# firstbatchxyz/dnet

Measured on AMD Instinct MI355X. Metric: output tokens/sec (whole node), qwen-2.5-32b int8 pipelined ring, higher is better.
Workload: dtype int8-g128 weights (bf16 compute); 1 GPU; model=qwen-2.5-32b, global_batch=64, seq_len=128, gen_len=178, parallelism=ring-pp1, microbatches=1, mb_size=64, layers=64

## Files before the change

dnet_amd/ops/csrc/gemm_m16.hip.cpp:

```cpp
#include "common.h"

namespace dnet {

using bf16x8 = __attribute__((ext_vector_type(8))) __bf16;
using f32x4 = __attribute__((ext_vector_type(4))) float;

__device__ __forceinline__ bf16x8 deq8(const int8_t* q, const float s) {
  bf16x8 b;
#pragma unroll
  for (int j = 0; j < 8; ++j) b[j] = (__bf16)((float)q[j] * s);
  return b;
}

__device__ __forceinline__ bf16x8 deq4(const uint8_t* qb, const float s) {
  bf16x8 b;
#pragma unroll
  for (int j = 0; j < 4; ++j) {
    const int byte = qb[j];
    b[2 * j] = (__bf16)((float)((byte & 0xF) - 8) * s);
    b[2 * j + 1] = (__bf16)((float)((byte >> 4) - 8) * s);
  }
  return b;
}

__device__ __forceinline__ float splitk_grid(const float v) {
  return rintf(v * 65536.0f) * (1.0f / 65536.0f);
}

template <int QBITS, int MT>
__global__ void gemm_m16_kernel(const short* __restrict__ x,
                                const void* __restrict__ w,
                                const short* __restrict__ scales,
                                const short* __restrict__ bias,
                                short* __restrict__ out,
                                float* __restrict__ out_f32,
                                const int M, const int K, const int N,
                                const int G, const int splitk,
                                const int exact) {
  constexpr int XT = 1024 / MT;
  constexpr int SE = XT + 8;
  __shared__ short x_lds[16 * MT * SE];
  const int wave = threadIdx.x / kWave;
  const int lane = threadIdx.x & (kWave - 1);
  const int n0 = (blockIdx.x * 4 + wave) * 16;
  const int row = lane & 15;
  const int ks = (lane >> 4) * 8;
  const int n_w = min(n0 + row, N - 1);

  const int pairs = K / 64;
  int p_begin, p_end;
  if (QBITS == 4) {
    const int quads = K / 128;
    const int qq = quads / splitk;
    p_begin = blockIdx.y * qq * 2;
    p_end = (blockIdx.y == splitk - 1) ? quads * 2 : p_begin + qq * 2;
  } else {
    const int pp = pairs / splitk;
    p_begin = blockIdx.y * pp;
    p_end = (blockIdx.y == splitk - 1) ? pairs : p_begin + pp;
  }
  const int woff = (lane >> 4) * 16;

  f32x4 acc[MT][2];
#pragma unroll
  for (int t = 0; t < MT; ++t)
#pragma unroll
    for (int u = 0; u < 2; ++u) acc[t][u] = {0.f, 0.f, 0.f, 0.f};

  const int8_t* wrow_q = (const int8_t*)w + (int64_t)n_w * K;
  const uint8_t* wrow_q4 = (const uint8_t*)w + (int64_t)n_w * (K / 2);
  const short* wrow_b = (const short*)w + (int64_t)n_w * K;
  const short* srow = QBITS < 16 ? scales + (int64_t)n_w * (K / G) : nullptr;

  for (int k0 = p_begin * 64; k0 < p_end * 64; k0 += XT) {
    const int tk = min(XT, p_end * 64 - k0);
    asm volatile("s_waitcnt lgkmcnt(0)" ::: "memory");
    asm volatile("s_barrier" ::: "memory");
    for (int idx = threadIdx.x; idx < 16 * MT * (tk / 8); idx += 256) {
      const int r = idx / (tk / 8);
      const int vec = idx % (tk / 8);
      *reinterpret_cast<short8*>(&x_lds[r * SE + vec * 8]) =
          *reinterpret_cast<const short8*>(
              &x[(int64_t)min(r, M - 1) * K + k0 + vec * 8]);
    }
    asm volatile("s_waitcnt lgkmcnt(0)" ::: "memory");
    asm volatile("s_barrier" ::: "memory");
    const short* arow = &x_lds[row * SE];
    int pl = 0;
    const int pl_end = tk / 64;
    for (; pl + 4 <= pl_end; pl += 4) {
      int4 wq8[4];
      int4 wq4[2];
      bf16x8 wb[4][2];
      float sv[4];
      if (QBITS == 8) {
#pragma unroll
        for (int u = 0; u < 4; ++u) {
          const int p = (k0 / 64) + pl + u;
          wq8[u] = *reinterpret_cast<const int4*>(&wrow_q[p * 64 + woff]);
          sv[u] = bits2f(srow[(p * 64) / G]);
        }
      } else if (QBITS == 4) {
#pragma unroll
        for (int v = 0; v < 2; ++v) {
          const int quad = ((k0 / 64) + pl) / 2 + v;
          wq4[v] = *reinterpret_cast<const int4*>(&wrow_q4[quad * 64 + woff]);
          sv[v] = bits2f(srow[(quad * 128) / G]);
        }
      } else {
#pragma unroll
        for (int u = 0; u < 4; ++u) {
          const int p = (k0 / 64) + pl + u;
          wb[u][0] = *reinterpret_cast<const bf16x8*>(&wrow_b[p * 64 + ks]);
          wb[u][1] = *reinterpret_cast<const bf16x8*>(
              &wrow_b[p * 64 + 32 + ks]);
        }
      }
#pragma unroll
      for (int u = 0; u < 4; ++u) {
        bf16x8 b0, b1;
        if (QBITS == 8) {
          const int8_t* q8 = reinterpret_cast<const int8_t*>(&wq8[u]);
          b0 = deq8(q8, sv[u]);
          b1 = deq8(q8 + 8, sv[u]);
        } else if (QBITS == 4) {
          const uint8_t* q4 =
              reinterpret_cast<const uint8_t*>(&wq4[u / 2]) + (u & 1) * 8;
          b0 = deq4(q4, sv[u / 2]);
          b1 = deq4(q4 + 4, sv[u / 2]);
        } else {
          b0 = wb[u][0];
          b1 = wb[u][1];
        }
#pragma unroll
        for (int t = 0; t < MT; ++t) {
          const short* at = arow + t * 16 * SE;
          const bf16x8 a0 =
              *reinterpret_cast<const bf16x8*>(&at[(pl + u) * 64 + ks]);
          const bf16x8 a1 =
              *reinterpret_cast<const bf16x8*>(&at[(pl + u) * 64 + 32 + ks]);
          acc[t][0] = __builtin_amdgcn_mfma_f32_16x16x32_bf16(
              a0, b0, acc[t][0], 0, 0, 0);
          acc[t][1] = __builtin_amdgcn_mfma_f32_16x16x32_bf16(
              a1, b1, acc[t][1], 0, 0, 0);
        }
      }
    }
    for (; pl < pl_end; ++pl) {
      const int p = (k0 / 64) + pl;
      bf16x8 b0, b1;
      if (QBITS == 8) {
        const int4 wq = *reinterpret_cast<const int4*>(&wrow_q[p * 64 + woff]);
        const int8_t* q8 = reinterpret_cast<const int8_t*>(&wq);
        const float sv = bits2f(srow[(p * 64) / G]);
        b0 = deq8(q8, sv);
        b1 = deq8(q8 + 8, sv);
      } else if (QBITS == 4) {
        const int quad = p / 2;
        const int half = p & 1;
        const int2 wq = *reinterpret_cast<const int2*>(
            &wrow_q4[quad * 64 + woff + half * 8]);
        const uint8_t* q4 = reinterpret_cast<const uint8_t*>(&wq);
        const float sv = bits2f(srow[(quad * 128) / G]);
        b0 = deq4(q4, sv);
        b1 = deq4(q4 + 4, sv);
      } else {
        b0 = *reinterpret_cast<const bf16x8*>(&wrow_b[p * 64 + ks]);
        b1 = *reinterpret_cast<const bf16x8*>(&wrow_b[p * 64 + 32 + ks]);
      }
#pragma unroll
      for (int t = 0; t < MT; ++t) {
        const short* at = arow + t * 16 * SE;
        const bf16x8 a0 = *reinterpret_cast<const bf16x8*>(&at[pl * 64 + ks]);
        const bf16x8 a1 = *reinterpret_cast<const bf16x8*>(&at[pl * 64 + 32 + ks]);
        acc[t][0] = __builtin_amdgcn_mfma_f32_16x16x32_bf16(a0, b0, acc[t][0],
                                                            0, 0, 0);
        acc[t][1] = __builtin_amdgcn_mfma_f32_16x16x32_bf16(a1, b1, acc[t][1],
                                                            0, 0, 0);
      }
    }
  }

  const int n = n0 + (lane & 15);
  if (n >= N) return;
#pragma unroll
  for (int t = 0; t < MT; ++t) {
    const f32x4 a2 = acc[t][0] + acc[t][1];
#pragma unroll
    for (int r = 0; r < 4; ++r) {
      const int m = t * 16 + (lane >> 4) * 4 + r;
      if (m >= M) continue;
      if (splitk > 1) {
        atomicAdd(out_f32 + (int64_t)m * N + n,
                  exact ? splitk_grid(a2[r]) : a2[r]);
      } else {
        float v = a2[r];
        if (bias != nullptr) v += bits2f(bias[n]);
        out[(int64_t)m * N + n] = f2bits(v);
      }
    }
  }
}


using i32x4 = __attribute__((ext_vector_type(4))) int;

template <int QBITS, int NSC>
struct WSet {
  i32x4 w[QBITS == 8 ? 4 : 2];
  unsigned s[NSC];
};

template <int QBITS, int NSC>
__device__ __forceinline__ void wset_load(WSet<QBITS, NSC>& o,
                                          const void* wb, const short* sb) {
  if constexpr (QBITS == 8 && NSC == 2) {
    asm volatile(
        "global_load_dwordx4 %0, %6, off\n\t"
        "global_load_dwordx4 %1, %6, off offset:64\n\t"
        "global_load_dwordx4 %2, %6, off offset:128\n\t"
        "global_load_dwordx4 %3, %6, off offset:192\n\t"
        "global_load_ushort %4, %7, off\n\t"
        "global_load_ushort %5, %7, off offset:2\n\t"
        "s_waitcnt vmcnt(0)"
        : "=&v"(o.w[0]), "=&v"(o.w[1]), "=&v"(o.w[2]), "=&v"(o.w[3]),
          "=&v"(o.s[0]), "=&v"(o.s[1])
        : "v"(wb), "v"(sb)
        : "memory");
  } else if constexpr (QBITS == 8 && NSC == 4) {
    asm volatile(
        "global_load_dwordx4 %0, %8, off\n\t"
        "global_load_dwordx4 %1, %8, off offset:64\n\t"
        "global_load_dwordx4 %2, %8, off offset:128\n\t"
        "global_load_dwordx4 %3, %8, off offset:192\n\t"
        "global_load_ushort %4, %9, off\n\t"
        "global_load_ushort %5, %9, off offset:2\n\t"
        "global_load_ushort %6, %9, off offset:4\n\t"
        "global_load_ushort %7, %9, off offset:6\n\t"
        "s_waitcnt vmcnt(0)"
        : "=&v"(o.w[0]), "=&v"(o.w[1]), "=&v"(o.w[2]), "=&v"(o.w[3]),
          "=&v"(o.s[0]), "=&v"(o.s[1]), "=&v"(o.s[2]), "=&v"(o.s[3])
        : "v"(wb), "v"(sb)
        : "memory");
  } else {
    static_assert(QBITS == 4 && NSC == 2, "unsupported stream variant");
    asm volatile(
        "global_load_dwordx4 %0, %4, off\n\t"
        "global_load_dwordx4 %1, %4, off offset:64\n\t"
        "global_load_ushort %2, %5, off\n\t"
        "global_load_ushort %3, %5, off offset:2\n\t"
        "s_waitcnt vmcnt(0)"
        : "=&v"(o.w[0]), "=&v"(o.w[1]), "=&v"(o.s[0]), "=&v"(o.s[1])
        : "v"(wb), "v"(sb)
        : "memory");
  }
}

template <int QBITS, int NSC>
struct WSet2 {
  i32x4 w[QBITS == 8 ? 8 : 4];
  unsigned s[2 * NSC];
};

template <int QBITS, int NSC>
__device__ __forceinline__ void wset_load2(WSet2<QBITS, NSC>& o,
                                           const void* wb, const short* sb) {
  if constexpr (QBITS == 8 && NSC == 2) {
    asm volatile(
        "global_load_dwordx4 %0, %12, off\n\t"
        "global_load_dwordx4 %1, %12, off offset:64\n\t"
        "global_load_dwordx4 %2, %12, off offset:128\n\t"
        "global_load_dwordx4 %3, %12, off offset:192\n\t"
        "global_load_dwordx4 %4, %12, off offset:256\n\t"
        "global_load_dwordx4 %5, %12, off offset:320\n\t"
        "global_load_dwordx4 %6, %12, off offset:384\n\t"
        "global_load_dwordx4 %7, %12, off offset:448\n\t"
        "global_load_ushort %8, %13, off\n\t"
        "global_load_ushort %9, %13, off offset:2\n\t"
        "global_load_ushort %10, %13, off offset:4\n\t"
        "global_load_ushort %11, %13, off offset:6\n\t"
        "s_waitcnt vmcnt(0)"
        : "=&v"(o.w[0]), "=&v"(o.w[1]), "=&v"(o.w[2]), "=&v"(o.w[3]),
          "=&v"(o.w[4]), "=&v"(o.w[5]), "=&v"(o.w[6]), "=&v"(o.w[7]),
          "=&v"(o.s[0]), "=&v"(o.s[1]), "=&v"(o.s[2]), "=&v"(o.s[3])
        : "v"(wb), "v"(sb)
        : "memory");
  } else if constexpr (QBITS == 8 && NSC == 4) {
    asm volatile(
        "global_load_dwordx4 %0, %16, off\n\t"
        "global_load_dwordx4 %1, %16, off offset:64\n\t"
        "global_load_dwordx4 %2, %16, off offset:128\n\t"
        "global_load_dwordx4 %3, %16, off offset:192\n\t"
        "global_load_dwordx4 %4, %16, off offset:256\n\t"
        "global_load_dwordx4 %5, %16, off offset:320\n\t"
        "global_load_dwordx4 %6, %16, off offset:384\n\t"
        "global_load_dwordx4 %7, %16, off offset:448\n\t"
        "global_load_ushort %8, %17, off\n\t"
        "global_load_ushort %9, %17, off offset:2\n\t"
        "global_load_ushort %10, %17, off offset:4\n\t"
        "global_load_ushort %11, %17, off offset:6\n\t"
        "global_load_ushort %12, %17, off offset:8\n\t"
        "global_load_ushort %13, %17, off offset:10\n\t"
        "global_load_ushort %14, %17, off offset:12\n\t"
        "global_load_ushort %15, %17, off offset:14\n\t"
        "s_waitcnt vmcnt(0)"
        : "=&v"(o.w[0]), "=&v"(o.w[1]), "=&v"(o.w[2]), "=&v"(o.w[3]),
          "=&v"(o.w[4]), "=&v"(o.w[5]), "=&v"(o.w[6]), "=&v"(o.w[7]),
          "=&v"(o.s[0]), "=&v"(o.s[1]), "=&v"(o.s[2]), "=&v"(o.s[3]),
          "=&v"(o.s[4]), "=&v"(o.s[5]), "=&v"(o.s[6]), "=&v"(o.s[7])
        : "v"(wb), "v"(sb)
        : "memory");
  } else {
    static_assert(QBITS == 4 && NSC == 2, "unsupported stream variant");
    asm volatile(
        "global_load_dwordx4 %0, %8, off\n\t"
        "global_load_dwordx4 %1, %8, off offset:64\n\t"
        "global_load_dwordx4 %2, %8, off offset:128\n\t"
        "global_load_dwordx4 %3, %8, off offset:192\n\t"
        "global_load_ushort %4, %9, off\n\t"
        "global_load_ushort %5, %9, off offset:2\n\t"
        "global_load_ushort %6, %9, off offset:4\n\t"
        "global_load_ushort %7, %9, off offset:6\n\t"
        "s_waitcnt vmcnt(0)"
        : "=&v"(o.w[0]), "=&v"(o.w[1]), "=&v"(o.w[2]), "=&v"(o.w[3]),
          "=&v"(o.s[0]), "=&v"(o.s[1]), "=&v"(o.s[2]), "=&v"(o.s[3])
        : "v"(wb), "v"(sb)
        : "memory");
  }
}

template <int MT, bool GLDS>
__device__ __forceinline__ void stage_tile(const short* __restrict__ x,
                                           short* x_lds, const int k0,
                                           const int M, const int K) {
  constexpr int NSG = MT * 2;
  asm volatile("s_waitcnt lgkmcnt(0)" ::: "memory");
  asm volatile("s_barrier" ::: "memory");
  const int wavei = (int)threadIdx.x >> 6, lanei = (int)threadIdx.x & 63;
  if constexpr (GLDS) {
#pragma unroll
    for (int g = 0; g < NSG; ++g) {
      const int L = (wavei * NSG + g) * 64 + lanei;
      const int r = L >> 5;
      const int cs = (L & 31) ^ (r & 15);
      const short* ga = &x[(int64_t)min(r, M - 1) * K + k0 + cs * 8];
      __builtin_amdgcn_global_load_lds(
          (const __attribute__((address_space(1))) void*)ga,
          (__attribute__((address_space(3))) void*)&x_lds[(wavei * NSG + g) *
                                                          64 * 8],
          16, 0, 0);
    }
  } else {
#pragma unroll
    for (int g = 0; g < NSG; ++g) {
      const int L = (wavei * NSG + g) * 64 + lanei;
      const int r = L >> 5;
      const int cs = (L & 31) ^ (r & 15);
      *reinterpret_cast<short8*>(&x_lds[L * 8]) =
          *reinterpret_cast<const short8*>(
              &x[(int64_t)min(r, M - 1) * K + k0 + cs * 8]);
    }
  }
}

template <bool GLDS>
__device__ __forceinline__ void end_stage() {
  asm volatile("s_waitcnt lgkmcnt(0)" ::: "memory");
  asm volatile("s_barrier" ::: "memory");
  if constexpr (GLDS)
    asm volatile("s_mov_b32 m0, -1" ::: "memory");
}

template <int QBITS, int MT, int NSC>
__device__ __forceinline__ void consume_tile(const i32x4* __restrict__ wv,
                                             const unsigned* __restrict__ sc,
                                             short* x_lds,
                                             f32x4 (&acc)[MT][2],
                                             const int row, const int ks) {
  const int ln4 = ks >> 3;
#pragma unroll
  for (int u = 0; u < 4; ++u) {
    bf16x8 b0, b1;
    if (QBITS == 8) {
      const int8_t* q8 = reinterpret_cast<const int8_t*>(&wv[u]);
      const float sv = bits2f((short)sc[u * NSC / 4]);
      b0 = deq8(q8, sv);
      b1 = deq8(q8 + 8, sv);
    } else {
      const uint8_t* q4 =
          reinterpret_cast<const uint8_t*>(&wv[u / 2]) + (u & 1) * 8;
      const float sv = bits2f((short)sc[(u / 2) * NSC / 2]);
      b0 = deq4(q4, sv);
      b1 = deq4(q4 + 4, sv);
    }
    const int c0 = (u * 8 + ln4) ^ row;
    const int c1 = (u * 8 + 4 + ln4) ^ row;
#pragma unroll
    for (int t = 0; t < MT; ++t) {
      const short* rb = &x_lds[(t * 16 + row) * 256];
      const bf16x8 a0 = *reinterpret_cast<const bf16x8*>(&rb[c0 * 8]);
      const bf16x8 a1 = *reinterpret_cast<const bf16x8*>(&rb[c1 * 8]);
      acc[t][0] =
          __builtin_amdgcn_mfma_f32_16x16x32_bf16(a0, b0, acc[t][0], 0, 0, 0);
      acc[t][1] =
          __builtin_amdgcn_mfma_f32_16x16x32_bf16(a1, b1, acc[t][1], 0, 0, 0);
    }
  }
}

template <int QBITS, int MT, int NSC, int MINW, bool GLDS = true>
__global__ __launch_bounds__(256, MINW) void gemm_m16_stream_kernel(
    const short* __restrict__ x, const void* __restrict__ w,
    const short* __restrict__ scales, const short* __restrict__ bias,
    short* __restrict__ out, float* __restrict__ out_f32, const int M,
    const int K, const int N, const int G, const int splitk,
    const int exact) {
  constexpr int XT = 256;
  __shared__ short x_lds[16 * MT * XT];
  const int wave = threadIdx.x / kWave;
  const int lane = threadIdx.x & (kWave - 1);
  const int n0 = (blockIdx.x * 4 + wave) * 16;
  const int row = lane & 15;
  const int ks = (lane >> 4) * 8;
  const int n_w = min(n0 + row, N - 1);

  const int pairs = K / 64;
  int p_begin, p_end;
  if (QBITS == 4) {
    const int quads = K / 128;
    const int qq = quads / splitk;
    p_begin = blockIdx.y * qq * 2;
    p_end = (blockIdx.y == splitk - 1) ? quads * 2 : p_begin + qq * 2;
  } else {
    const int pp = pairs / splitk;
    p_begin = blockIdx.y * pp;
    p_end = (blockIdx.y == splitk - 1) ? pairs : p_begin + pp;
  }
  const int woff = (lane >> 4) * 16;

  f32x4 acc[MT][2];
#pragma unroll
  for (int t = 0; t < MT; ++t)
#pragma unroll
    for (int u = 0; u < 2; ++u) acc[t][u] = {0.f, 0.f, 0.f, 0.f};

  const void* wrow =
      QBITS == 8
          ? (const void*)((const int8_t*)w + (int64_t)n_w * K + woff)
          : (const void*)((const uint8_t*)w + (int64_t)n_w * (K / 2) + woff);
  const short* srow = scales + (int64_t)n_w * (K / G);

  const int kbeg = p_begin * 64, kend = p_end * 64;
  const int kfull = kbeg + ((kend - kbeg) / XT) * XT;
  constexpr int GS = 256 / NSC;
  int k0 = kbeg;
  for (; k0 + 2 * XT <= kfull; k0 += 2 * XT) {
    WSet2<QBITS, NSC> w2;
    stage_tile<MT, GLDS>(x, x_lds, k0, M, K);
    if (QBITS == 8)
      wset_load2<QBITS, NSC>(w2, (const int8_t*)wrow + k0, srow + k0 / GS);
    else
      wset_load2<QBITS, NSC>(w2, (const uint8_t*)wrow + k0 / 2,
                             srow + k0 / GS);
    end_stage<GLDS>();
    consume_tile<QBITS, MT, NSC>(&w2.w[0], &w2.s[0], x_lds, acc, row, ks);
    stage_tile<MT, GLDS>(x, x_lds, k0 + XT, M, K);
    asm volatile("s_waitcnt vmcnt(0)" ::: "memory");
    end_stage<GLDS>();
    consume_tile<QBITS, MT, NSC>(&w2.w[QBITS == 8 ? 4 : 2], &w2.s[NSC],
                                 x_lds, acc, row, ks);
  }
  for (; k0 < kfull; k0 += XT) {
    WSet<QBITS, NSC> w1;
    stage_tile<MT, GLDS>(x, x_lds, k0, M, K);
    if (QBITS == 8)
      wset_load<QBITS, NSC>(w1, (const int8_t*)wrow + k0, srow + k0 / GS);
    else
      wset_load<QBITS, NSC>(w1, (const uint8_t*)wrow + k0 / 2,
                            srow + k0 / GS);
    end_stage<GLDS>();
    consume_tile<QBITS, MT, NSC>(&w1.w[0], &w1.s[0], x_lds, acc, row, ks);
  }

  const int ln4 = ks >> 3;
  for (; k0 < kend; k0 += XT) {
    const int tk = kend - k0;
    asm volatile("s_waitcnt lgkmcnt(0)" ::: "memory");
    asm volatile("s_barrier" ::: "memory");
    for (int idx = threadIdx.x; idx < 16 * MT * (tk / 8); idx += 256) {
      const int r = idx / (tk / 8);
      const int vec = idx % (tk / 8);
      *reinterpret_cast<short8*>(&x_lds[(r * 32 + (vec ^ (r & 15))) * 8]) =
          *reinterpret_cast<const short8*>(
              &x[(int64_t)min(r, M - 1) * K + k0 + vec * 8]);
    }
    asm volatile("s_waitcnt lgkmcnt(0)" ::: "memory");
    asm volatile("s_barrier" ::: "memory");
    for (int pl = 0; pl < tk / 64; ++pl) {
      const int p = (k0 / 64) + pl;
      bf16x8 b0, b1;
      if (QBITS == 8) {
        const int8_t* wq = (const int8_t*)wrow;
        const int4 wv = *reinterpret_cast<const int4*>(&wq[p * 64]);
        const int8_t* q8 = reinterpret_cast<const int8_t*>(&wv);
        const float sv = bits2f(srow[(p * 64) / G]);
        b0 = deq8(q8, sv);
        b1 = deq8(q8 + 8, sv);
      } else {
        const int quad = p / 2;
        const int half = p & 1;
        const uint8_t* wq = (const uint8_t*)wrow;
        const int2 wv =
            *reinterpret_cast<const int2*>(&wq[quad * 64 + half * 8]);
        const uint8_t* q4 = reinterpret_cast<const uint8_t*>(&wv);
        const float sv = bits2f(srow[(quad * 128) / G]);
        b0 = deq4(q4, sv);
        b1 = deq4(q4 + 4, sv);
      }
      const int c0 = (pl * 8 + ln4) ^ row;
      const int c1 = (pl * 8 + 4 + ln4) ^ row;
#pragma unroll
      for (int t = 0; t < MT; ++t) {
        const short* rb = &x_lds[(t * 16 + row) * 256];
        const bf16x8 a0 = *reinterpret_cast<const bf16x8*>(&rb[c0 * 8]);
        const bf16x8 a1 = *reinterpret_cast<const bf16x8*>(&rb[c1 * 8]);
        acc[t][0] = __builtin_amdgcn_mfma_f32_16x16x32_bf16(a0, b0, acc[t][0],
                                                            0, 0, 0);
        acc[t][1] = __builtin_amdgcn_mfma_f32_16x16x32_bf16(a1, b1, acc[t][1],
                                                            0, 0, 0);
      }
    }
  }

  const int n = n0 + (lane & 15);
  if (n >= N) return;
#pragma unroll
  for (int t = 0; t < MT; ++t) {
    const f32x4 a2 = acc[t][0] + acc[t][1];
#pragma unroll
    for (int r = 0; r < 4; ++r) {
      const int m = t * 16 + (lane >> 4) * 4 + r;
      if (m >= M) continue;
      if (splitk > 1) {
        atomicAdd(out_f32 + (int64_t)m * N + n,
                  exact ? splitk_grid(a2[r]) : a2[r]);
      } else {
        float v = a2[r];
        if (bias != nullptr) v += bits2f(bias[n]);
        out[(int64_t)m * N + n] = f2bits(v);
      }
    }
  }
}

__global__ void f32_to_bf16_bias_kernel(const float* __restrict__ in,
                                        const short* __restrict__ bias,
                                        short* __restrict__ out,
                                        const int64_t total, const int N) {
  for (int64_t i = blockIdx.x * (int64_t)blockDim.x + threadIdx.x; i < total;
       i += (int64_t)gridDim.x * blockDim.x) {
    float v = in[i];
    if (bias != nullptr) v += bits2f(bias[i % N]);
    out[i] = f2bits(v);
  }
}

static int64_t g_scratch_dirty_elems = 0;

static bool g_splitk_exact = false;
void set_splitk_exact(bool on) { g_splitk_exact = on; }

static int pick_splitk(int64_t N, int64_t K, int64_t M, int64_t scratch_elems,
                       int min_pairs, int g_align) {
  static const int forced = []() {
    const char* e = getenv("DNET_GEMM_SPLITK");
    return e ? atoi(e) : 0;
  }();
  const int blocks = (int)((N + 63) / 64);
  if (forced > 0)
    return (M * N > scratch_elems || (K / 64) < forced) ? 1 : forced;
  int sk = 1;
  while (sk < 32 && blocks * sk < 1024 &&
         (K / 64) / (sk * 2) >= min_pairs &&
         ((K / 64) / (sk * 2)) * 64 % g_align == 0)
    sk *= 2;
  if (sk > 1) {
    const int64_t span = ((K / 64) / sk) * 64;
    const int64_t span2 = ((K / 64) / (sk / 2)) * 64;
    if (span % 256 != 0 && (double)(span % 256) / span >= 0.15 &&
        span2 % 256 == 0 && span2 % g_align == 0 &&
        blocks * (sk / 2) >= 440)
      sk /= 2;
  }
  if (sk > 1 && M * N > scratch_elems) sk = 1;
  return sk;
}

static bool launch_m16(torch::Tensor x, torch::Tensor w,
                       c10::optional<torch::Tensor> scales,
                       c10::optional<torch::Tensor> bias, torch::Tensor out,
                       c10::optional<torch::Tensor> scratch, int group,
                       int64_t m0, int M, int bits, bool defer_combine) {
  const int64_t K = x.size(1), N = w.size(0);
  auto stream = current_stream();
  const int64_t scratch_elems = scratch.has_value() ? scratch->numel() : 0;
  const int sk = pick_splitk(N, K, M, scratch_elems, bits < 16 ? 4 : 8,
                             bits < 16 ? std::max<int>((int)group, 64) : 64);
  const short* bptr = bias.has_value() ? (const short*)bias->data_ptr() : nullptr;
  const dim3 grid((unsigned)((N + 63) / 64), sk);
  const int exact = g_splitk_exact ? 1 : 0;
  const short* xp = (const short*)x.data_ptr() + m0 * K;
  short* op = (short*)out.data_ptr() + m0 * N;
  float* fp = nullptr;
  if (sk > 1) {
    TORCH_CHECK(scratch.has_value() && scratch->numel() >= (int64_t)M * N,
                "split-k scratch required");
    fp = (float*)scratch->data_ptr();
    if (g_scratch_dirty_elems > 0) {
      const int64_t span = std::max<int64_t>(g_scratch_dirty_elems,
                                             (int64_t)M * N);
      DNET_CHECK_HIP(hipMemsetAsync(fp, 0, sizeof(float) * span, stream));
      g_scratch_dirty_elems = 0;
    }
  }
  const short* sp = bits < 16 ? (const short*)scales->data_ptr() : nullptr;
  const short* bp1 = sk > 1 ? nullptr : bptr;
#define LAUNCH(QQ, TT)                                                      \
  hipLaunchKernelGGL((gemm_m16_kernel<QQ, TT>), grid, dim3(256), 0, stream, \
                     xp, w.data_ptr(), sp, bp1, op, fp, M, (int)K, (int)N,  \
                     group, sk, exact)
  static const bool mt4occ3 = []() {
    const char* e = getenv("DNET_GEMM_MT4OCC");
    return e == nullptr || e[0] == '3';
  }();
  static const bool noglds = getenv("DNET_GEMM_NOGLDS") != nullptr;
#define LAUNCH_STREAM(QQ, TT, NSC, MW)                                      \
  do {                                                                      \
    if (noglds)                                                             \
      hipLaunchKernelGGL((gemm_m16_stream_kernel<QQ, TT, NSC, MW, false>), \
                         grid, dim3(256), 0, stream, xp, w.data_ptr(), sp,  \
                         bp1, op, fp, M, (int)K, (int)N, group, sk, exact); \
    else                                                                    \
      hipLaunchKernelGGL((gemm_m16_stream_kernel<QQ, TT, NSC, MW, true>),   \
                         grid, dim3(256), 0, stream, xp, w.data_ptr(), sp,  \
                         bp1, op, fp, M, (int)K, (int)N, group, sk, exact); \
  } while (0)
#define LAUNCH_STREAM_G8(TT)                                            \
  do {                                                                    \
    if (TT == 4 && mt4occ3) {                                             \
      if (group == 64) LAUNCH_STREAM(8, TT, 4, 3);                        \
      else LAUNCH_STREAM(8, TT, 2, 3);                                    \
    } else {                                                              \
      if (group == 64) LAUNCH_STREAM(8, TT, 4, 4);                        \
      else LAUNCH_STREAM(8, TT, 2, 4);                                    \
    }                                                                     \
  } while (0)
#define LAUNCH_STREAM_G4(TT)                                              \
  do {                                                                    \
    if (TT == 4 && mt4occ3) LAUNCH_STREAM(4, TT, 2, 3);                   \
    else LAUNCH_STREAM(4, TT, 2, 4);                                      \
  } while (0)
  const bool split_aligned =
      group > 0 && (sk == 1 || ((K / 64 / sk) * 64) % group == 0);
  const bool can_stream =
      split_aligned && ((bits == 8 && (group == 64 || group == 128)) ||
                        (bits == 4 && group == 128));
  static const bool nostream = getenv("DNET_GEMM_NOSTREAM") != nullptr;
  const bool use_stream = can_stream && !nostream;
  if (bits == 8) {
    if (M > 32) { if (use_stream) LAUNCH_STREAM_G8(4); else LAUNCH(8, 4); }
    else if (M > 16) { if (use_stream) LAUNCH_STREAM_G8(2); else LAUNCH(8, 2); }
    else { if (use_stream) LAUNCH_STREAM_G8(1); else LAUNCH(8, 1); }
  } else if (bits == 4) {
    if (M > 32) { if (use_stream) LAUNCH_STREAM_G4(4); else LAUNCH(4, 4); }
    else if (M > 16) { if (use_stream) LAUNCH_STREAM_G4(2); else LAUNCH(4, 2); }
    else { if (use_stream) LAUNCH_STREAM_G4(1); else LAUNCH(4, 1); }
  } else {
    if (M > 32) LAUNCH(16, 4);
    else if (M > 16) LAUNCH(16, 2);
    else LAUNCH(16, 1);
  }
#undef LAUNCH
#undef LAUNCH_STREAM
#undef LAUNCH_STREAM_G8
#undef LAUNCH_STREAM_G4
  if (sk > 1) {
    if (defer_combine && bptr == nullptr) return true;
    const int64_t total = (int64_t)M * N;
    const int cgrid = (int)std::min<int64_t>((total + 255) / 256, 2048);
    hipLaunchKernelGGL(f32_to_bf16_bias_kernel, dim3(cgrid), dim3(256), 0,
                       stream, fp, bptr, op, total, (int)N);
    g_scratch_dirty_elems =
        std::max<int64_t>(g_scratch_dirty_elems, (int64_t)M * N);
  }
  return false;
}

bool gemm_m16_will_defer(int64_t M, int64_t N, int64_t K, int64_t group,
                         int64_t bits, int64_t scratch_elems) {
  if (M > 64 || M <= 2) return false;
  const int sk = pick_splitk(N, K, M, scratch_elems, bits < 16 ? 4 : 8,
                             bits < 16 ? std::max<int>((int)group, 64) : 64);
  return sk > 1;
}

bool gemm_m16(torch::Tensor x, torch::Tensor w,
              c10::optional<torch::Tensor> scales,
              c10::optional<torch::Tensor> bias, torch::Tensor out,
              c10::optional<torch::Tensor> scratch, int64_t group,
              bool packed, int64_t bits, bool defer_combine) {
  const int64_t M = x.size(0), K = x.size(1), N = w.size(0);
  DNET_CHECK(K % 64 == 0, "K % 64 == 0 required for the MFMA path");
  DNET_CHECK(out.size(0) == M && out.size(1) == N, "shape");
  DNET_CHECK(x.is_contiguous() && w.is_contiguous() && out.is_contiguous(), "contig");
  if (bits == 16) {
    DNET_CHECK(w.size(1) == K, "w shape");
  } else {
    DNET_CHECK(packed, "quantized MFMA path expects the packed weight layout");
    DNET_CHECK(scales.has_value() && scales->is_contiguous(), "scales");
    DNET_CHECK(group % 64 == 0 && K % group == 0, "group align");
    if (bits == 8) DNET_CHECK(w.size(1) == K, "w shape (int8)");
    if (bits == 4) {
      DNET_CHECK(w.size(1) == K / 2 && K % 128 == 0 && group % 128 == 0,
                 "w shape / align (int4)");
    }
  }
  const bool defer = defer_combine && M <= 64 && !bias.has_value();
  bool deferred = false;
  int64_t m0 = 0;
  while (m0 < M) {
    const int mt = (int)std::min<int64_t>(M - m0, 64);
    deferred = launch_m16(x, w, scales, bias, out, scratch, (int)group, m0,
                          mt, (int)bits, defer);
    m0 += mt;
  }
  return deferred;
}

}
```

Measured before the change: 3782 tokens/s.

## Double-buffer activation tiles and weight registers in streaming int8 GEMM kernel

Rewrites the streaming dequant GEMM main loop as a software pipeline: two LDS images of the activation tile and two weight register sets, so the next tile's global loads are issued before the current tile's MFMA work. Inside each tile, fragment reads and dequantization for the next sub-step are interleaved with the MFMAs using scheduling barriers. The partial-tail path is folded into the same pipelined code, and group size becomes a compile-time template parameter. This doubles LDS use and raises register pressure, and the occupancy hint is lowered accordingly, which could reduce latency hiding across waves.

```diff
diff --git a/dnet_amd/ops/csrc/gemm_m16.hip.cpp b/dnet_amd/ops/csrc/gemm_m16.hip.cpp
--- a/dnet_amd/ops/csrc/gemm_m16.hip.cpp
+++ b/dnet_amd/ops/csrc/gemm_m16.hip.cpp
@@ -205,223 +205,138 @@
 
 using i32x4 = __attribute__((ext_vector_type(4))) int;
 
-template <int QBITS, int NSC>
+constexpr int kWaitVm0 = 0x0F70;
+constexpr int kWaitLgkm0 = 0xC07F;
+
+template <int QBITS, int G, int XT>
 struct WSet {
-  i32x4 w[QBITS == 8 ? 4 : 2];
-  unsigned s[NSC];
+  static constexpr int NW = QBITS == 8 ? XT / 64 : XT / 128;
+  static constexpr int NS = XT / G;
+  i32x4 w[NW];
+  unsigned s[NS];
 };
 
-template <int QBITS, int NSC>
-__device__ __forceinline__ void wset_load(WSet<QBITS, NSC>& o,
-                                          const void* wb, const short* sb) {
-  if constexpr (QBITS == 8 && NSC == 2) {
-    asm volatile(
-        "global_load_dwordx4 %0, %6, off\n\t"
-        "global_load_dwordx4 %1, %6, off offset:64\n\t"
-        "global_load_dwordx4 %2, %6, off offset:128\n\t"
-        "global_load_dwordx4 %3, %6, off offset:192\n\t"
-        "global_load_ushort %4, %7, off\n\t"
-        "global_load_ushort %5, %7, off offset:2\n\t"
-        "s_waitcnt vmcnt(0)"
-        : "=&v"(o.w[0]), "=&v"(o.w[1]), "=&v"(o.w[2]), "=&v"(o.w[3]),
-          "=&v"(o.s[0]), "=&v"(o.s[1])
-        : "v"(wb), "v"(sb)
-        : "memory");
-  } else if constexpr (QBITS == 8 && NSC == 4) {
-    asm volatile(
-        "global_load_dwordx4 %0, %8, off\n\t"
-        "global_load_dwordx4 %1, %8, off offset:64\n\t"
-        "global_load_dwordx4 %2, %8, off offset:128\n\t"
-        "global_load_dwordx4 %3, %8, off offset:192\n\t"
-        "global_load_ushort %4, %9, off\n\t"
-        "global_load_ushort %5, %9, off offset:2\n\t"
-        "global_load_ushort %6, %9, off offset:4\n\t"
-        "global_load_ushort %7, %9, off offset:6\n\t"
-        "s_waitcnt vmcnt(0)"
-        : "=&v"(o.w[0]), "=&v"(o.w[1]), "=&v"(o.w[2]), "=&v"(o.w[3]),
-          "=&v"(o.s[0]), "=&v"(o.s[1]), "=&v"(o.s[2]), "=&v"(o.s[3])
-        : "v"(wb), "v"(sb)
-        : "memory");
-  } else {
-    static_assert(QBITS == 4 && NSC == 2, "unsupported stream variant");
-    asm volatile(
-        "global_load_dwordx4 %0, %4, off\n\t"
-        "global_load_dwordx4 %1, %4, off offset:64\n\t"
-        "global_load_ushort %2, %5, off\n\t"
-        "global_load_ushort %3, %5, off offset:2\n\t"
-        "s_waitcnt vmcnt(0)"
-        : "=&v"(o.w[0]), "=&v"(o.w[1]), "=&v"(o.s[0]), "=&v"(o.s[1])
-        : "v"(wb), "v"(sb)
-        : "memory");
-  }
-}
-
-template <int QBITS, int NSC>
-struct WSet2 {
-  i32x4 w[QBITS == 8 ? 8 : 4];
-  unsigned s[2 * NSC];
-};
-
-template <int QBITS, int NSC>
-__device__ __forceinline__ void wset_load2(WSet2<QBITS, NSC>& o,
-                                           const void* wb, const short* sb) {
-  if constexpr (QBITS == 8 && NSC == 2) {
-    asm volatile(
-        "global_load_dwordx4 %0, %12, off\n\t"
-        "global_load_dwordx4 %1, %12, off offset:64\n\t"
-        "global_load_dwordx4 %2, %12, off offset:128\n\t"
-        "global_load_dwordx4 %3, %12, off offset:192\n\t"
-        "global_load_dwordx4 %4, %12, off offset:256\n\t"
-        "global_load_dwordx4 %5, %12, off offset:320\n\t"
-        "global_load_dwordx4 %6, %12, off offset:384\n\t"
-        "global_load_dwordx4 %7, %12, off offset:448\n\t"
-        "global_load_ushort %8, %13, off\n\t"
-        "global_load_ushort %9, %13, off offset:2\n\t"
-        "global_load_ushort %10, %13, off offset:4\n\t"
-        "global_load_ushort %11, %13, off offset:6\n\t"
-        "s_waitcnt vmcnt(0)"
-        : "=&v"(o.w[0]), "=&v"(o.w[1]), "=&v"(o.w[2]), "=&v"(o.w[3]),
-          "=&v"(o.w[4]), "=&v"(o.w[5]), "=&v"(o.w[6]), "=&v"(o.w[7]),
-          "=&v"(o.s[0]), "=&v"(o.s[1]), "=&v"(o.s[2]), "=&v"(o.s[3])
-        : "v"(wb), "v"(sb)
-        : "memory");
-  } else if constexpr (QBITS == 8 && NSC == 4) {
-    asm volatile(
-        "global_load_dwordx4 %0, %16, off\n\t"
-        "global_load_dwordx4 %1, %16, off offset:64\n\t"
-        "global_load_dwordx4 %2, %16, off offset:128\n\t"
-        "global_load_dwordx4 %3, %16, off offset:192\n\t"
-        "global_load_dwordx4 %4, %16, off offset:256\n\t"
-        "global_load_dwordx4 %5, %16, off offset:320\n\t"
-        "global_load_dwordx4 %6, %16, off offset:384\n\t"
-        "global_load_dwordx4 %7, %16, off offset:448\n\t"
-        "global_load_ushort %8, %17, off\n\t"
-        "global_load_ushort %9, %17, off offset:2\n\t"
-        "global_load_ushort %10, %17, off offset:4\n\t"
-        "global_load_ushort %11, %17, off offset:6\n\t"
-        "global_load_ushort %12, %17, off offset:8\n\t"
-        "global_load_ushort %13, %17, off offset:10\n\t"
-        "global_load_ushort %14, %17, off offset:12\n\t"
-        "global_load_ushort %15, %17, off offset:14\n\t"
-        "s_waitcnt vmcnt(0)"
-        : "=&v"(o.w[0]), "=&v"(o.w[1]), "=&v"(o.w[2]), "=&v"(o.w[3]),
-          "=&v"(o.w[4]), "=&v"(o.w[5]), "=&v"(o.w[6]), "=&v"(o.w[7]),
-          "=&v"(o.s[0]), "=&v"(o.s[1]), "=&v"(o.s[2]), "=&v"(o.s[3]),
-          "=&v"(o.s[4]), "=&v"(o.s[5]), "=&v"(o.s[6]), "=&v"(o.s[7])
-        : "v"(wb), "v"(sb)
-        : "memory");
-  } else {
-    static_assert(QBITS == 4 && NSC == 2, "unsupported stream variant");
-    asm volatile(
-        "global_load_dwordx4 %0, %8, off\n\t"
-        "global_load_dwordx4 %1, %8, off offset:64\n\t"
-        "global_load_dwordx4 %2, %8, off offset:128\n\t"
-        "global_load_dwordx4 %3, %8, off offset:192\n\t"
-        "global_load_ushort %4, %9, off\n\t"
-        "global_load_ushort %5, %9, off offset:2\n\t"
-        "global_load_ushort %6, %9, off offset:4\n\t"
-        "global_load_ushort %7, %9, off offset:6\n\t"
-        "s_waitcnt vmcnt(0)"
-        : "=&v"(o.w[0]), "=&v"(o.w[1]), "=&v"(o.w[2]), "=&v"(o.w[3]),
-          "=&v"(o.s[0]), "=&v"(o.s[1]), "=&v"(o.s[2]), "=&v"(o.s[3])
-        : "v"(wb), "v"(sb)
-        : "memory");
-  }
-}
-
-template <int MT, bool GLDS>
-__device__ __forceinline__ void stage_tile(const short* __restrict__ x,
-                                           short* x_lds, const int k0,
-                                           const int M, const int K) {
-  constexpr int NSG = MT * 2;
-  asm volatile("s_waitcnt lgkmcnt(0)" ::: "memory");
-  asm volatile("s_barrier" ::: "memory");
+template <int QBITS, int G, int XT, bool FULL>
+__device__ __forceinline__ void wset_load(WSet<QBITS, G, XT>& o,
+                                          const char* wb,
+                                          const unsigned short* sb,
+                                          const int np) {
+  constexpr int PPW = QBITS == 8 ? 1 : 2;
+#pragma unroll
+  for (int v = 0; v < WSet<QBITS, G, XT>::NW; ++v) {
+    if (FULL || v * PPW < np)
+      o.w[v] = *reinterpret_cast<const i32x4*>(wb + v * 64);
+    else
+      o.w[v] = i32x4{0, 0, 0, 0};
+  }
+#pragma unroll
+  for (int j = 0; j < WSet<QBITS, G, XT>::NS; ++j)
+    o.s[j] = (FULL || j * G < np * 64) ? (unsigned)sb[j] : 0u;
+}
+
+template <int MT, int XT, bool GLDS>
+__device__ __forceinline__ void stage_tile(const short* __restrict__ xk,
+                                           short* img,
+                                           const unsigned (&offb)[MT * XT / 128]) {
+  constexpr int NSG = MT * XT / 128;
   const int wavei = (int)threadIdx.x >> 6, lanei = (int)threadIdx.x & 63;
   if constexpr (GLDS) {
-#pragma unroll
-    for (int g = 0; g < NSG; ++g) {
-      const int L = (wavei * NSG + g) * 64 + lanei;
-      const int r = L >> 5;
-      const int cs = (L & 31) ^ (r & 15);
-      const short* ga = &x[(int64_t)min(r, M - 1) * K + k0 + cs * 8];
-      __builtin_amdgcn_global_load_lds(
-          (const __attribute__((address_space(1))) void*)ga,
-          (__attribute__((address_space(3))) void*)&x_lds[(wavei * NSG + g) *
-                                                          64 * 8],
-          16, 0, 0);
-    }
+    const unsigned base = __builtin_amdgcn_readfirstlane(
+        (unsigned)(unsigned long)(__attribute__((address_space(3))) short*)img +
+        (unsigned)wavei * NSG * 1024u);
+#pragma unroll
+    for (int g = 0; g < NSG; ++g)
+      asm volatile(
+          "s_mov_b32 m0, %0\n\t"
+          "s_nop 0\n\t"
+          "global_load_lds_dwordx4 %1, %2"
+          :
+          : "s"(base + g * 1024u), "v"(offb[g]), "s"(xk)
+          : "memory");
+    asm volatile("s_mov_b32 m0, -1" ::: "memory");
   } else {
 #pragma unroll
-    for (int g = 0; g < NSG; ++g) {
-      const int L = (wavei * NSG + g) * 64 + lanei;
-      const int r = L >> 5;
-      const int cs = (L & 31) ^ (r & 15);
-      *reinterpret_cast<short8*>(&x_lds[L * 8]) =
-          *reinterpret_cast<const short8*>(
-              &x[(int64_t)min(r, M - 1) * K + k0 + cs * 8]);
-    }
-  }
-}
-
-template <bool GLDS>
-__device__ __forceinline__ void end_stage() {
-  asm volatile("s_waitcnt lgkmcnt(0)" ::: "memory");
-  asm volatile("s_barrier" ::: "memory");
-  if constexpr (GLDS)
-    asm volatile("s_mov_b32 m0, -1" ::: "memory");
-}
-
-template <int QBITS, int MT, int NSC>
-__device__ __forceinline__ void consume_tile(const i32x4* __restrict__ wv,
-                                             const unsigned* __restrict__ sc,
-                                             short* x_lds,
+    for (int g = 0; g < NSG; ++g)
+      *reinterpret_cast<short8*>(&img[((wavei * NSG + g) * 64 + lanei) * 8]) =
+          *reinterpret_cast<const short8*>((const char*)xk + offb[g]);
+  }
+}
+
+template <int QBITS, int MT, int G, int XT, bool FULL>
+__device__ __forceinline__ void consume_tile(const WSet<QBITS, G, XT>& ws,
+                                             const short* img,
                                              f32x4 (&acc)[MT][2],
-                                             const int row, const int ks) {
-  const int ln4 = ks >> 3;
-#pragma unroll
-  for (int u = 0; u < 4; ++u) {
-    bf16x8 b0, b1;
+                                             const int row, const int ln4,
+                                             const int np) {
+  constexpr int PT = XT / 64;
+  const short* rb = img + row * XT;
+  int v = ln4 ^ row;
+  asm volatile("" : "+v"(v));
+  bf16x8 a[2][MT][2];
+  bf16x8 b[2][2];
+  auto frag = [&](const int u, const int s) __attribute__((always_inline)) {
+#pragma unroll
+    for (int t = 0; t < MT; ++t) {
+      a[s][t][0] = *reinterpret_cast<const bf16x8*>(
+          &rb[t * 16 * XT + ((u * 8) ^ v) * 8]);
+      a[s][t][1] = *reinterpret_cast<const bf16x8*>(
+          &rb[t * 16 * XT + ((u * 8 + 4) ^ v) * 8]);
+    }
+  };
+  auto deq = [&](const int u, const int s) __attribute__((always_inline)) {
+    const float sv = bits2f((short)ws.s[u * 64 / G]);
+    i32x4 wq = ws.w[QBITS == 8 ? u : u / 2];
+    asm volatile("" : "+v"(wq));
     if (QBITS == 8) {
-      const int8_t* q8 = reinterpret_cast<const int8_t*>(&wv[u]);
-      const float sv = bits2f((short)sc[u * NSC / 4]);
-      b0 = deq8(q8, sv);
-      b1 = deq8(q8 + 8, sv);
+      const int8_t* q8 = reinterpret_cast<const int8_t*>(&wq);
+      b[s][0] = deq8(q8, sv);
+      b[s][1] = deq8(q8 + 8, sv);
     } else {
-      const uint8_t* q4 =
-          reinterpret_cast<const uint8_t*>(&wv[u / 2]) + (u & 1) * 8;
-      const float sv = bits2f((short)sc[(u / 2) * NSC / 2]);
-      b0 = deq4(q4, sv);
-      b1 = deq4(q4 + 4, sv);
-    }
-    const int c0 = (u * 8 + ln4) ^ row;
-    const int c1 = (u * 8 + 4 + ln4) ^ row;
+      const uint8_t* q4 = reinterpret_cast<const uint8_t*>(&wq) + (u & 1) * 8;
+      b[s][0] = deq4(q4, sv);
+      b[s][1] = deq4(q4 + 4, sv);
+    }
+  };
+  frag(0, 0);
+  __builtin_amdgcn_sched_barrier(0);
+  deq(0, 0);
+#pragma unroll
+  for (int u = 0; u < PT; ++u) {
+    if (!FULL && u >= np) break;
+    const int s = u & 1;
+    if (u + 1 < PT && (FULL || u + 1 < np)) frag(u + 1, s ^ 1);
+    __builtin_amdgcn_sched_barrier(0);
+    if (u + 1 < PT) deq(u + 1, s ^ 1);
 #pragma unroll
     for (int t = 0; t < MT; ++t) {
-      const short* rb = &x_lds[(t * 16 + row) * 256];
-      const bf16x8 a0 = *reinterpret_cast<const bf16x8*>(&rb[c0 * 8]);
-      const bf16x8 a1 = *reinterpret_cast<const bf16x8*>(&rb[c1 * 8]);
-      acc[t][0] =
-          __builtin_amdgcn_mfma_f32_16x16x32_bf16(a0, b0, acc[t][0], 0, 0, 0);
-      acc[t][1] =
-          __builtin_amdgcn_mfma_f32_16x16x32_bf16(a1, b1, acc[t][1], 0, 0, 0);
-    }
-  }
-}
-
-template <int QBITS, int MT, int NSC, int MINW, bool GLDS = true>
+      acc[t][0] = __builtin_amdgcn_mfma_f32_16x16x32_bf16(
+          a[s][t][0], b[s][0], acc[t][0], 0, 0, 0);
+      acc[t][1] = __builtin_amdgcn_mfma_f32_16x16x32_bf16(
+          a[s][t][1], b[s][1], acc[t][1], 0, 0, 0);
+    }
+    __builtin_amdgcn_sched_barrier(0);
+  }
+}
+
+template <int QBITS, int MT, int G, int XT, int MINW, bool GLDS = true>
 __global__ __launch_bounds__(256, MINW) void gemm_m16_stream_kernel(
     const short* __restrict__ x, const void* __restrict__ w,
     const short* __restrict__ scales, const short* __restrict__ bias,
     short* __restrict__ out, float* __restrict__ out_f32, const int M,
-    const int K, const int N, const int G, const int splitk,
-    const int exact) {
-  constexpr int XT = 256;
-  __shared__ short x_lds[16 * MT * XT];
+    const int K, const int N, const int splitk, const int exact) {
+  using WS = WSet<QBITS, G, XT>;
+  constexpr int PT = XT / 64;
+  constexpr int CPR = XT / 8;
+  constexpr int NSG = MT * XT / 128;
+  constexpr int TILE = 16 * MT * XT;
+  __shared__ short x_lds[2 * TILE];
+  short* const x_img0 = x_lds;
+  short* const x_img1 = x_lds + TILE;
   const int wave = threadIdx.x / kWave;
   const int lane = threadIdx.x & (kWave - 1);
   const int n0 = (blockIdx.x * 4 + wave) * 16;
   const int row = lane & 15;
-  const int ks = (lane >> 4) * 8;
+  const int ln4 = lane >> 4;
   const int n_w = min(n0 + row, N - 1);
 
   const int pairs = K / 64;
@@ -436,7 +351,7 @@
     p_begin = blockIdx.y * pp;
     p_end = (blockIdx.y == splitk - 1) ? pairs : p_begin + pp;
   }
-  const int woff = (lane >> 4) * 16;
+  const int woff = ln4 * 16;
 
   f32x4 acc[MT][2];
 #pragma unroll
@@ -444,91 +359,71 @@
 #pragma unroll
     for (int u = 0; u < 2; ++u) acc[t][u] = {0.f, 0.f, 0.f, 0.f};
 
-  const void* wrow =
-      QBITS == 8
-          ? (const void*)((const int8_t*)w + (int64_t)n_w * K + woff)
-          : (const void*)((const uint8_t*)w + (int64_t)n_w * (K / 2) + woff);
-  const short* srow = scales + (int64_t)n_w * (K / G);
+  const char* wrow = (const char*)w +
+                     (int64_t)n_w * (QBITS == 8 ? K : K / 2) + woff;
+  const unsigned short* srow =
+      (const unsigned short*)scales + (int64_t)n_w * (K / G);
 
   const int kbeg = p_begin * 64, kend = p_end * 64;
-  const int kfull = kbeg + ((kend - kbeg) / XT) * XT;
-  constexpr int GS = 256 / NSC;
-  int k0 = kbeg;
-  for (; k0 + 2 * XT <= kfull; k0 += 2 * XT) {
-    WSet2<QBITS, NSC> w2;
-    stage_tile<MT, GLDS>(x, x_lds, k0, M, K);
-    if (QBITS == 8)
-      wset_load2<QBITS, NSC>(w2, (const int8_t*)wrow + k0, srow + k0 / GS);
+  const int nfull = (kend - kbeg) / XT;
+  const int rem = (kend - kbeg) - nfull * XT;
+  const int ntiles = nfull + (rem > 0 ? 1 : 0);
+
+  unsigned offb[NSG];
+#pragma unroll
+  for (int g = 0; g < NSG; ++g) {
+    const int L = (wave * NSG + g) * 64 + lane;
+    const int r = L / CPR;
+    const int cs8 = ((L % CPR) ^ (r & 15)) * 8;
+    offb[g] = 2u * (unsigned)(min(r, M - 1) * K + cs8);
+  }
+
+  auto issue = [&](const int i, short* img, WS& dst)
+      __attribute__((always_inline)) {
+    const int k0 = kbeg + i * XT;
+    const char* wb = wrow + (QBITS == 8 ? k0 : k0 / 2);
+    if (i < nfull) {
+      stage_tile<MT, XT, GLDS>(x + k0, img, offb);
+      wset_load<QBITS, G, XT, true>(dst, wb, srow + k0 / G, PT);
+    } else {
+      unsigned offp[NSG];
+#pragma unroll
+      for (int g = 0; g < NSG; ++g) {
+        const int L = (wave * NSG + g) * 64 + lane;
+        const int r = L / CPR;
+        const int cs8 = ((L % CPR) ^ (r & 15)) * 8;
+        offp[g] = 2u * (unsigned)(min(r, M - 1) * K + min(cs8, rem - 8));
+      }
+      stage_tile<MT, XT, GLDS>(x + k0, img, offp);
+      wset_load<QBITS, G, XT, false>(dst, wb, srow + k0 / G, rem / 64);
+    }
+    __builtin_amdgcn_sched_barrier(0);
+  };
+  auto step = [&](const int i, const short* img, short* img_next, WS& cur,
+                  WS& nxt) __attribute__((always_inline)) {
+    __builtin_amdgcn_s_waitcnt(kWaitLgkm0);
+    asm volatile("s_barrier" ::: "memory");
+    if (i + 1 < ntiles) issue(i + 1, img_next, nxt);
+    if (i < nfull)
+      consume_tile<QBITS, MT, G, XT, true>(cur, img, acc, row, ln4, PT);
     else
-      wset_load2<QBITS, NSC>(w2, (const uint8_t*)wrow + k0 / 2,
-                             srow + k0 / GS);
-    end_stage<GLDS>();
-    consume_tile<QBITS, MT, NSC>(&w2.w[0], &w2.s[0], x_lds, acc, row, ks);
-    stage_tile<MT, GLDS>(x, x_lds, k0 + XT, M, K);
-    asm volatile("s_waitcnt vmcnt(0)" ::: "memory");
-    end_stage<GLDS>();
-    consume_tile<QBITS, MT, NSC>(&w2.w[QBITS == 8 ? 4 : 2], &w2.s[NSC],
-                                 x_lds, acc, row, ks);
-  }
-  for (; k0 < kfull; k0 += XT) {
-    WSet<QBITS, NSC> w1;
-    stage_tile<MT, GLDS>(x, x_lds, k0, M, K);
-    if (QBITS == 8)
-      wset_load<QBITS, NSC>(w1, (const int8_t*)wrow + k0, srow + k0 / GS);
-    else
-      wset_load<QBITS, NSC>(w1, (const uint8_t*)wrow + k0 / 2,
-                            srow + k0 / GS);
-    end_stage<GLDS>();
-    consume_tile<QBITS, MT, NSC>(&w1.w[0], &w1.s[0], x_lds, acc, row, ks);
-  }
-
-  const int ln4 = ks >> 3;
-  for (; k0 < kend; k0 += XT) {
-    const int tk = kend - k0;
-    asm volatile("s_waitcnt lgkmcnt(0)" ::: "memory");
-    asm volatile("s_barrier" ::: "memory");
-    for (int idx = threadIdx.x; idx < 16 * MT * (tk / 8); idx += 256) {
-      const int r = idx / (tk / 8);
-      const int vec = idx % (tk / 8);
-      *reinterpret_cast<short8*>(&x_lds[(r * 32 + (vec ^ (r & 15))) * 8]) =
-          *reinterpret_cast<const short8*>(
-              &x[(int64_t)min(r, M - 1) * K + k0 + vec * 8]);
-    }
-    asm volatile("s_waitcnt lgkmcnt(0)" ::: "memory");
-    asm volatile("s_barrier" ::: "memory");
-    for (int pl = 0; pl < tk / 64; ++pl) {
-      const int p = (k0 / 64) + pl;
-      bf16x8 b0, b1;
-      if (QBITS == 8) {
-        const int8_t* wq = (const int8_t*)wrow;
-        const int4 wv = *reinterpret_cast<const int4*>(&wq[p * 64]);
-        const int8_t* q8 = reinterpret_cast<const int8_t*>(&wv);
-        const float sv = bits2f(srow[(p * 64) / G]);
-        b0 = deq8(q8, sv);
-        b1 = deq8(q8 + 8, sv);
-      } else {
-        const int quad = p / 2;
-        const int half = p & 1;
-        const uint8_t* wq = (const uint8_t*)wrow;
-        const int2 wv =
-            *reinterpret_cast<const int2*>(&wq[quad * 64 + half * 8]);
-        const uint8_t* q4 = reinterpret_cast<const uint8_t*>(&wv);
-        const float sv = bits2f(srow[(quad * 128) / G]);
-        b0 = deq4(q4, sv);
-        b1 = deq4(q4 + 4, sv);
-      }
-      const int c0 = (pl * 8 + ln4) ^ row;
-      const int c1 = (pl * 8 + 4 + ln4) ^ row;
-#pragma unroll
-      for (int t = 0; t < MT; ++t) {
-        const short* rb = &x_lds[(t * 16 + row) * 256];
-        const bf16x8 a0 = *reinterpret_cast<const bf16x8*>(&rb[c0 * 8]);
-        const bf16x8 a1 = *reinterpret_cast<const bf16x8*>(&rb[c1 * 8]);
-        acc[t][0] = __builtin_amdgcn_mfma_f32_16x16x32_bf16(a0, b0, acc[t][0],
-                                                            0, 0, 0);
-        acc[t][1] = __builtin_amdgcn_mfma_f32_16x16x32_bf16(a1, b1, acc[t][1],
-                                                            0, 0, 0);
-      }
+      consume_tile<QBITS, MT, G, XT, false>(cur, img, acc, row, ln4,
+                                             rem / 64);
+    __builtin_amdgcn_sched_barrier(0);
+    __builtin_amdgcn_s_waitcnt(kWaitVm0);
+  };
+
+  if (ntiles > 0) {
+    WS wa, wb2;
+#pragma unroll
+    for (int v = 0; v < WS::NW; ++v) wb2.w[v] = i32x4{0, 0, 0, 0};
+#pragma unroll
+    for (int j = 0; j < WS::NS; ++j) wb2.s[j] = 0u;
+    issue(0, x_img0, wa);
+    __builtin_amdgcn_s_waitcnt(kWaitVm0);
+    for (int i = 0; i < ntiles; i += 2) {
+      step(i, x_img0, x_img1, wa, wb2);
+      if (i + 1 < ntiles) step(i + 1, x_img1, x_img0, wb2, wa);
     }
   }
 
@@ -629,37 +524,28 @@
   hipLaunchKernelGGL((gemm_m16_kernel<QQ, TT>), grid, dim3(256), 0, stream, \
                      xp, w.data_ptr(), sp, bp1, op, fp, M, (int)K, (int)N,  \
                      group, sk, exact)
-  static const bool mt4occ3 = []() {
-    const char* e = getenv("DNET_GEMM_MT4OCC");
-    return e == nullptr || e[0] == '3';
-  }();
   static const bool noglds = getenv("DNET_GEMM_NOGLDS") != nullptr;
-#define LAUNCH_STREAM(QQ, TT, NSC, MW)                                      \
+#define LAUNCH_STREAM(QQ, TT, GG, XT, MW)                                   \
   do {                                                                      \
     if (noglds)                                                             \
-      hipLaunchKernelGGL((gemm_m16_stream_kernel<QQ, TT, NSC, MW, false>), \
-                         grid, dim3(256), 0, stream, xp, w.data_ptr(), sp,  \
-                         bp1, op, fp, M, (int)K, (int)N, group, sk, exact); \
+      hipLaunchKernelGGL(                                                   \
+          (gemm_m16_stream_kernel<QQ, TT, GG, XT, 2, false>), grid,         \
+          dim3(256), 0, stream, xp, w.data_ptr(), sp, bp1, op, fp, M,       \
+          (int)K, (int)N, sk, exact);                                       \
     else                                                                    \
-      hipLaunchKernelGGL((gemm_m16_stream_kernel<QQ, TT, NSC, MW, true>),   \
-                         grid, dim3(256), 0, stream, xp, w.data_ptr(), sp,  \
-                         bp1, op, fp, M, (int)K, (int)N, group, sk, exact); \
+      hipLaunchKernelGGL(                                                   \
+          (gemm_m16_stream_kernel<QQ, TT, GG, XT, MW, true>), grid,         \
+          dim3(256), 0, stream, xp, w.data_ptr(), sp, bp1, op, fp, M,       \
+          (int)K, (int)N, sk, exact);                                       \
   } while (0)
-#define LAUNCH_STREAM_G8(TT)                                            \
-  do {                                                                    \
-    if (TT == 4 && mt4occ3) {                                             \
-      if (group == 64) LAUNCH_STREAM(8, TT, 4, 3);                        \
-      else LAUNCH_STREAM(8, TT, 2, 3);                                    \
-    } else {                                                              \
-      if (group == 64) LAUNCH_STREAM(8, TT, 4, 4);                        \
-      else LAUNCH_STREAM(8, TT, 2, 4);                                    \
-    }                                                                     \
+#define LAUNCH_STREAM_T(QQ, TT, GG) \
+  LAUNCH_STREAM(QQ, TT, GG, 256, (TT == 4 ? 2 : TT == 2 ? 3 : 4))
+#define LAUNCH_STREAM_G8(TT)                                                \
+  do {                                                                      \
+    if (group == 64) LAUNCH_STREAM_T(8, TT, 64);                            \
+    else LAUNCH_STREAM_T(8, TT, 128);                                       \
   } while (0)
-#define LAUNCH_STREAM_G4(TT)                                              \
-  do {                                                                    \
-    if (TT == 4 && mt4occ3) LAUNCH_STREAM(4, TT, 2, 3);                   \
-    else LAUNCH_STREAM(4, TT, 2, 4);                                      \
-  } while (0)
+#define LAUNCH_STREAM_G4(TT) LAUNCH_STREAM_T(4, TT, 128)
   const bool split_aligned =
       group > 0 && (sk == 1 || ((K / 64 / sk) * 64) % group == 0);
   const bool can_stream =
@@ -682,6 +568,7 @@
   }
 #undef LAUNCH
 #undef LAUNCH_STREAM
+#undef LAUNCH_STREAM_T
 #undef LAUNCH_STREAM_G8
 #undef LAUNCH_STREAM_G4
   if (sk > 1) {
```

Measured after the change: 3869 tokens/s, median of 6. +2.3%, better.
